# koadman/libMems

Measured on AMD Instinct MI355X. Metric: seed-mers/sec sorted+matched (+ MUMs/sec) at 1/2/4/8 MI355X; HBM GB/s vs roofline, higher is better.
Workload: dtype u64; 1 GPU; BASELINE config 3: 8 x 100 Mbp, seed weight 19 (0x7b974ef), MemHash seed stage (sorted+matched); genomes=8, genome_length=100000000, seedmers_total=799999792, seedmers_rank0=799999792, probes_rank0=100459493, parallelism=1 GPU

## Files before the change

libmems_amd/csrc/mums_internal.h:

```cpp
#pragma once

#include <hip/hip_runtime.h>
#include <stdint.h>
#include <stdlib.h>

#include <vector>

#include "restart_plan.h"

namespace mums {

constexpr int kMaxG = 64;
constexpr int kRepeatLimit = 1000;
constexpr int kBlock = 256;
#ifndef MUMS_SEED_TILE
#define MUMS_SEED_TILE 4096
#endif
constexpr int kSeedTile = MUMS_SEED_TILE;
#ifndef MUMS_SEG_TILE
#define MUMS_SEG_TILE 4096
#endif
constexpr int kSegTile = MUMS_SEG_TILE;
#ifndef MUMS_GROUP_SPLIT
#define MUMS_GROUP_SPLIT 2
#endif
#ifndef MUMS_PROBE_TAKE
#define MUMS_PROBE_TAKE 1984
#endif
constexpr int kProbeSplit = MUMS_GROUP_SPLIT;
constexpr int kProbeTake = MUMS_PROBE_TAKE;
constexpr int kProbeTile = kProbeSplit * kProbeTake;
static_assert(kSegTile % kProbeSplit == 0 && kProbeTake >= 2 && kProbeTake <= kSegTile / kProbeSplit,
              "a probe workgroup takes at most what it stages");
constexpr int kLocalIPT = 16;
constexpr int kMaxMsdBits = 11;
constexpr int kMaxSegBucketBits = 12;

constexpr int kMaxSeedRuns = 16;

struct SeedSpec {
    uint64_t pattern;
    int L;
    int w;
    int nruns;
    int run_start[32];
    int run_len[32];
    int run_dst[32];
    int run_sh[kMaxSeedRuns];
    uint64_t run_mask[kMaxSeedRuns];
};

struct GenomeTable {
    int G;
    uint64_t n[kMaxG];
    uint64_t m[kMaxG];
    uint64_t base[kMaxG + 1];
    uint64_t woff[kMaxG + 1];
    uint32_t tfirst[kMaxG + 1];
    uint32_t gl_shift;
    uint32_t gl_n;
    uint8_t gl[256];
};

inline void genome_lookup_init(GenomeTable& gt) {
    gt.gl_n = 0;
    gt.gl_shift = 0;
    const uint64_t N = gt.base[gt.G];
    if (gt.G < 2 || N == 0 || N >= (1ull << 32)) return;
    if (getenv("MUMS_DEV_NO_GL")) return;
    uint64_t mn = ~0ull;
    for (int g = 0; g < gt.G; ++g) mn = gt.m[g] < mn ? gt.m[g] : mn;
    if (mn == 0) return;
    const int sh = 63 - __builtin_clzll(mn);
    const uint64_t nb = ((N - 1) >> sh) + 1;
    if (nb > 256) return;
    int g = 0;
    for (uint64_t s = 0; s < nb; ++s) {
        const uint64_t i = s << sh;
        while (g + 1 < gt.G && gt.base[g + 1] <= i) ++g;
        gt.gl[s] = (uint8_t)g;
    }
    gt.gl_shift = (uint32_t)sh;
    gt.gl_n = (uint32_t)nb;
}

struct MatchParams {
    uint32_t repeat_tol;
    uint32_t enum_tol;
    uint32_t table_size;
    int masked;
    uint64_t seq_mask;
};

struct DevCounters {
    unsigned long long groups;
    unsigned long long repeat_limit;
    unsigned long long collisions;
    unsigned long long entries;
    uint32_t err;
    uint32_t ntiles;
    uint32_t nprobes;
    uint32_t nmatches;
    uint32_t ngroups;
    uint32_t nchains;
    uint32_t max_bucket;
    uint32_t scratch32;
    unsigned long long walk_words;
    unsigned long long walk_items;
    unsigned long long walk_wins;
    unsigned long long short_words;
    unsigned long long short_items;
    unsigned long long short_wins;
    unsigned long long log_n;
    unsigned long long row_total;
};

struct SegTile {
    uint64_t start;
    uint64_t bstart;
    uint64_t bend;
    uint32_t count;
    uint32_t hbase;
    uint32_t ntb;
    uint32_t tb;
    uint32_t bucket;
    uint32_t order;
};

template <int kBits>
__device__ __forceinline__ uint32_t wave_match_rank_from(uint32_t dg, uint32_t pl, uint32_t ph, uint32_t* peers_out) {
    #pragma unroll
    for (int b = 0; b < kBits; ++b) {
        const uint32_t ms = (uint32_t)__builtin_amdgcn_sbfe((int32_t)dg, b, 1);
        const uint64_t x = __builtin_amdgcn_uicmp(ms, 0u, 33);
        pl = __builtin_amdgcn_bitop3_b32(pl, (uint32_t)x, ms, 0x90);
        ph = __builtin_amdgcn_bitop3_b32(ph, (uint32_t)(x >> 32), ms, 0x90);
    }
    *peers_out = (uint32_t)__builtin_popcount(pl) + (uint32_t)__builtin_popcount(ph);
    return __builtin_amdgcn_mbcnt_hi(ph, __builtin_amdgcn_mbcnt_lo(pl, 0u));
}

template <int kBits>
__device__ __forceinline__ uint32_t wave_match_rank(uint32_t dg, bool valid, uint32_t* peers_out) {
    const uint64_t v = __ballot(valid);
    return wave_match_rank_from<kBits>(dg, (uint32_t)v, (uint32_t)(v >> 32), peers_out);
}

template <int kBits>
__device__ __forceinline__ uint32_t wave_match_rank(uint32_t dg, uint32_t* peers_out) {
    return wave_match_rank_from<kBits>(dg, 0xFFFFFFFFu, 0xFFFFFFFFu, peers_out);
}

__device__ __forceinline__ uint64_t compat_gid(uint64_t k, int kbits) {
    return ((k >> 1) & 0x3FFFFFFFull) | (((k >> kbits) & 1ull) << 30);
}

__device__ __forceinline__ int genome_of(const GenomeTable& gt, uint64_t i) {
    int g = 0;
    #pragma unroll 1
    for (int k = 1; k < gt.G; ++k) g += (i >= gt.base[k]) ? 1 : 0;
    return g;
}

__host__ __device__ inline uint64_t packed_words(uint64_t n) { return (2 * n) / 32 + (((2 * n) % 32) ? 1 : 0) + 2; }

hipError_t launch_seed_pack(const SeedSpec& ss, const GenomeTable& gt, const char* const* d_ascii,
                            uint32_t* d_packed, int mode, bool key64, void* d_ckey, int msd_bits,
                            uint32_t* d_hist, uint32_t ntiles, uint32_t* d_err, hipStream_t st);
hipError_t launch_seed_scatter(const SeedSpec& ss, const GenomeTable& gt, const uint32_t* d_packed, int msd_bits,
                               const uint32_t* d_hist_scanned, uint32_t ntiles, uint64_t* d_rec, hipStream_t st,
                               uint8_t* d_side = nullptr, int side_bits = 0);
hipError_t launch_seed_scatter_chunk(const SeedSpec& ss, const GenomeTable& gt, const uint32_t* d_packed, int msd_bits,
                                     const uint32_t* d_hist_slice, uint32_t ntiles, uint32_t dlo, uint32_t nbc,
                                     uint64_t* d_rec, hipStream_t st, const uint64_t* d_cbase = nullptr, int mb = 0,
                                     uint8_t* d_side = nullptr, int side_bits = 0);
size_t msd_split_tmp_bytes(uint64_t n, int parent_bits);
hipError_t msd_split(const uint64_t* rin, const uint8_t* side, uint64_t* rout, uint64_t n, int parent_bits, int S,
                     const uint32_t* bstart_in, uint32_t* bstart_out, void* d_tmp, hipStream_t st);
hipError_t launch_keys_of_genome(const SeedSpec& ss, const uint32_t* d_words, uint64_t m, uint64_t* d_out,
                                 hipStream_t st, bool ref_form = true);

size_t scan_tmp_bytes(uint64_t n);
hipError_t exclusive_scan_u32(uint32_t* d_data, uint64_t n, void* d_tmp, uint32_t* d_total, hipStream_t st);
hipError_t launch_sum_u64(const uint32_t* d_data, uint64_t n, unsigned long long* d_total, hipStream_t st);

size_t radix_tmp_bytes(uint64_t n);
template <typename K>
hipError_t radix_sort(const K* keys_in, const uint32_t* vals_in, uint64_t n, int bits,
                      K* kA, uint32_t* vA, K* kB, uint32_t* vB, void* d_tmp, int* out_buf,
                      hipStream_t st, hipEvent_t* ev_ds = nullptr);

uint64_t seg_tiles_upper(uint64_t n, int msd_bits, uint32_t tile = kSegTile);
size_t seg_tmp_bytes(uint64_t n, int msd_bits);
hipError_t launch_regroup(const uint64_t* src, uint64_t* dst, const uint64_t* d_chunks, uint32_t nchunks, uint64_t n,
                          hipStream_t st);
hipError_t seg_bucket_starts(const uint32_t* d_hist_scanned, uint32_t T, int msd_bits, uint64_t n, uint32_t* bstart,
                             hipStream_t st);
hipError_t build_seg_tiles_from_starts(const uint32_t* bstart, int msd_bits, uint64_t n, SegTile* d_tiles,
                                       uint32_t* d_ntiles, void* d_tmp, hipStream_t st, uint32_t tile = kSegTile);
hipError_t build_seg_tiles(const uint32_t* d_hist_scanned, uint32_t T, int msd_bits, uint64_t n, SegTile* d_tiles,
                           uint32_t* d_ntiles, uint32_t* d_bstart, void* d_tmp, hipStream_t st);
hipError_t seg_radix_sort(uint64_t* recA, uint64_t* recB, uint64_t n, int key_bits, const SegTile* d_tiles,
                          uint64_t ntiles_ub, void* d_tmp, int* out_buf, hipStream_t st,
                          hipEvent_t* ev_ds = nullptr);
size_t onesweep_tmp_bytes(uint64_t n, int msd_bits, int key_bits);
hipError_t seg_onesweep_sort(uint64_t* recA, uint64_t* recB, uint64_t n, int key_bits, int msd_bits,
                             const uint32_t* d_bstart, void* d_tmp, uint32_t* d_err, int* out_buf, hipStream_t st,
                             hipEvent_t* ev_ds = nullptr, int key_shift = 32, bool mask_parity = false,
                             bool key_runs = false, const uint32_t* hist_in = nullptr,
                             const uint64_t* gsrc = nullptr, uint32_t* gout = nullptr);
size_t seg_parity_fix_tmp_bytes(uint64_t n);
hipError_t seg_parity_fix(uint64_t* rec, uint64_t* scratch, uint64_t n, int key_bits, int msd_bits,
                          const uint32_t* d_bstart, void* d_tmp, uint32_t* d_err, hipStream_t st, int key_shift = 32);
int seg_onesweep_launches(int key_bits);
bool seg_wide_sort_enabled();
int seg_wide_passes(int key_bits);
size_t onesweep_wide_tmp_bytes(uint64_t n, int msd_bits, int key_bits);
hipError_t seg_onesweep_sort_wide(uint64_t* recA, uint64_t* recB, uint64_t n, int key_bits, int msd_bits,
                                  const uint32_t* d_bstart, void* d_tmp, uint32_t* d_err, int* out_buf,
                                  hipStream_t st, hipEvent_t* ev_ds, int key_shift = 32);

inline uint64_t group_tiles_upper(uint64_t n, int msd_bits) { return seg_tiles_upper(n, msd_bits, kProbeTile); }
uint64_t group_slot_count(uint64_t ntiles);
uint64_t group_blocks(uint64_t ntiles, bool packed);
template <int MG, typename View>
hipError_t launch_probe_tiles(View v, const SegTile* tiles, uint64_t ntiles, uint64_t N, const GenomeTable& gt,
                              const MatchParams& mp, int L, uint32_t* tile_count, uint64_t* slot_info,
                              uint32_t* slot_bucket, void* counters, hipStream_t st);
hipError_t launch_probe_compact(uint64_t nblocks, const uint32_t* tile_count, const uint32_t* tile_off,
                                const uint64_t* slot_info, const uint32_t* slot_bucket, uint64_t* probe_info,
                                uint32_t* probe_bucket, hipStream_t st, bool packed);
template <int MG, typename View>
hipError_t launch_materialize(View v, const uint64_t* probe_info, uint64_t P, const GenomeTable& gt,
                              const MatchParams& mp, int L, int64_t* rows, hipStream_t st, uint64_t* lkey = nullptr,
                              uint32_t* fsk = nullptr, uint32_t* lhash = nullptr, int32_t* rows32 = nullptr);
hipError_t launch_row_buckets(const int64_t* rows, uint64_t P, int G, uint32_t table_size, const uint32_t* d_bounds,
                              uint32_t nranks, uint32_t* out, hipStream_t st);
hipError_t launch_gather_rows(const int64_t* src, const uint32_t* perm, uint64_t P, int G, int64_t* dst,
                              hipStream_t st);
hipError_t launch_rec_pairs(const uint64_t* rec, uint64_t n, const uint32_t* d_bst, uint32_t nb, uint32_t kfirst,
                            int kb_rec, uint64_t* key, uint32_t* idx, hipStream_t st);
hipError_t launch_rec_pairs33(const uint64_t* rec, uint64_t n, const uint32_t* d_bst, uint32_t nb, uint32_t kfirst,
                              int kb_rec, uint64_t* key, uint64_t* idx, hipStream_t st);
hipError_t launch_chain_dest(const uint32_t* fk, uint64_t nch, const uint32_t* pdest, uint32_t* cdest, hipStream_t st);
hipError_t launch_inverse_perm(const uint32_t* perm, uint64_t n, uint32_t* inv, hipStream_t st);
hipError_t launch_chain_tags(const uint32_t* chain_of, const uint32_t* perm, const uint32_t* sdest, uint64_t P,
                             const uint32_t* cinv, const uint32_t* cstart, uint32_t* tags, hipStream_t st);
hipError_t launch_chain_entries_out(const int64_t* pool, const uint32_t* fk, const uint32_t* cperm,
                                    const uint32_t* scdest, uint64_t nch, int G, const uint32_t* pinv,
                                    const uint32_t* rstart, int64_t* eout, uint32_t* fout, hipStream_t st);
hipError_t launch_kept_dest(const int64_t* rows, uint64_t P, int G, const uint32_t* chain_of, const uint32_t* cinv,
                            const uint2* thr, const uint32_t* fk, const uint32_t* pdest, uint32_t nranks, uint32_t* dest,
                            hipStream_t st);
hipError_t launch_dest_first(const uint32_t* sdest, uint64_t P, uint32_t* first, hipStream_t st);
hipError_t launch_entry_first(const uint32_t* scdest, uint64_t nch, const uint32_t* rcount, const uint32_t* perm,
                              const uint32_t* sdest, uint64_t K, const uint32_t* chain_of, const uint32_t* cinv,
                              const uint32_t* rstart, uint32_t* efirst, hipStream_t st);
hipError_t launch_flat_tiles(uint64_t N, SegTile* d_tiles, hipStream_t st, bool packed = false);
inline uint64_t flat_group_tiles(uint64_t N, bool packed) {
    const uint64_t tile = packed ? kProbeTile : kSegTile;
    return (N + tile - 1) / tile;
}

hipError_t launch_bucket_ranges(const uint32_t* sb, uint64_t P, uint32_t* bstart, uint32_t* bend, uint32_t* d_max,
                                hipStream_t st);
template <int MG, typename View>
hipError_t launch_replay_kept(View v, const GenomeTable& gt, const MatchParams& mp, int L, uint64_t P,
                              const int64_t* pool, const uint32_t* chain_of, const uint32_t* fk, uint32_t nch,
                              void* d_tmp, void* d_radix_tmp, void* d_scan_tmp, uint32_t lds_cap, uint32_t* tsize,
                              void* ctr, uint64_t* dbg, hipStream_t st, uint64_t* mlog, uint32_t** tbl_out,
                              const uint32_t** base_out, void* (*alloc)(void*, size_t), void* alloc_ctx,
                              const uint32_t* jl = nullptr);
template <int MG, typename View>
hipError_t launch_replay_carried(View v, const GenomeTable& gt, const MatchParams& mp, int L, uint64_t P,
                                 const int64_t* pool, uint32_t C, const uint32_t* kcnt, uint32_t nch,
                                 const uint32_t* jl, uint32_t lds_max, uint32_t* tsize, void* ctr, hipStream_t st,
                                 uint64_t* mlog, uint32_t** tbl_out, const uint32_t** base_out,
                                 void* (*alloc)(void*, size_t), void* alloc_ctx);
hipError_t launch_keep_pack(const uint64_t* len, const int64_t* s, uint64_t M, int G, int64_t* pool, hipStream_t st);
}
struct mums_ctx;
namespace mums {
hipStream_t ctx_stream(mums_ctx* ctx);
int ctx_device(mums_ctx* ctx);
int ctx_table_genomes(mums_ctx* ctx, uint32_t* table_size, uint32_t* genomes);
uint32_t ctx_repeat_tol(mums_ctx* ctx);
bool ctx_merge_chunked(mums_ctx* ctx);
bool ctx_tie_all(mums_ctx* ctx);
bool ctx_pcompat(mums_ctx* ctx);
int ctx_compat_layout(mums_ctx* ctx, uint32_t* first, uint32_t* nown, std::vector<uint64_t>* lens);
int ctx_compat_rank_find(mums_ctx* ctx, const char* const* d_ascii, const uint64_t* lens, int G, uint32_t rank,
                         uint32_t ranks, int stage);
int ctx_compat_rank_export(mums_ctx* ctx, uint64_t* bucket_counts, int64_t* d_rows, uint64_t* M);
int ctx_compat_rank_merge(mums_ctx* ctx, const int64_t* d_rows, uint32_t W, const uint64_t* counts, uint32_t nb);

struct EoWork {
    void *K = nullptr, *V = nullptr, *V2 = nullptr, *fl = nullptr, *fr = nullptr, *Lpos = nullptr, *Rpos = nullptr;
    void *bound = nullptr, *segA = nullptr, *segB = nullptr, *act = nullptr, *heap = nullptr, *piv = nullptr;
    void *nsw = nullptr, *scratch = nullptr, *plen = nullptr, *ps = nullptr, *nm_key = nullptr, *nm_id = nullptr;
    void *nk2 = nullptr, *nv2 = nullptr, *nk3 = nullptr, *nv3 = nullptr, *radix = nullptr, *ctr = nullptr;
    uint64_t cap_n = 0, cap_pool = 0, cap_new = 0, pool_n = 0, n_final = 0;
    int pool_G = 0;
    unsigned long long hbuf[8] = {};
    EoWork() = default;
    EoWork(const EoWork&) = delete;
    EoWork& operator=(const EoWork&) = delete;
    ~EoWork();
    void release();
};
hipError_t eliminate_overlaps_device(EoWork& w, const uint64_t* d_len, const int64_t* d_s, uint64_t M, int G,
                                     uint64_t* M_out, hipStream_t st);
hipError_t eliminate_overlaps_v2_device(EoWork& w, const uint64_t* d_len, const int64_t* d_s, uint64_t M, int G,
                                        const uint32_t* seq_ids, uint32_t nids, bool eliminate_both, uint64_t* M_out,
                                        hipStream_t st);
hipError_t eo_gather(EoWork& w, int G, uint64_t* d_len_out, int64_t* d_s_out, hipStream_t st);
hipError_t eo_sort_ids(EoWork& w, const uint64_t* d_keys, uint32_t n, int depth_override, uint32_t* d_ids_out,
                       hipStream_t st);

size_t chain_tmp_bytes(uint64_t P, uint32_t Tb, int G);
hipError_t launch_add_offset(uint32_t* a, uint64_t n, uint32_t off, hipStream_t st);
size_t chain_merge_tmp_bytes(uint64_t n);
size_t chain_thr_tmp_bytes(uint64_t n);
hipError_t launch_chain_thresholds(const int64_t* entries, uint64_t n, const GenomeTable& gt, const MatchParams& mp,
                                   int64_t* pool_out, void* d_tmp, void* d_radix_tmp, void* d_scan_tmp,
                                   uint32_t* d_nchains, uint32_t* h_nchains, uint2* thr, hipStream_t st);
hipError_t launch_chain_merge(const int64_t* pool_loc, uint64_t n, int G, uint32_t* chain_of, uint64_t P,
                              int64_t* pool_out, void* d_tmp, void* d_radix_tmp, void* d_scan_tmp, uint32_t* d_nchains,
                              hipStream_t st, const uint32_t* fk_loc, uint32_t* fk_out);
size_t chain_radix_tmp_bytes(uint64_t P);
template <int MG, typename View>
hipError_t launch_chains(View v, const uint64_t* probe_info, uint64_t P, const GenomeTable& gt, const MatchParams& mp,
                         const SeedSpec& ss, const uint32_t* packed, void* d_chain_tmp, void* d_scan_tmp,
                         void* d_radix_tmp, uint32_t* chain_of, int64_t* pool, uint32_t* d_nchains, hipStream_t st,
                         void* ctr, hipEvent_t* ev_walk, uint32_t* fk, uint32_t kbase, bool lkey_ready = false,
                         uint32_t* jl = nullptr);
uint64_t* chain_lkey_slot(void* d_chain_tmp, uint64_t P, int G);
bool chain_line_records(uint64_t P, const GenomeTable& gt);
void chain_line_slots(void* d_chain_tmp, uint64_t P, int G, uint64_t** rec, uint32_t** lhash);
hipError_t launch_emit(const uint32_t* obase, const uint32_t* bstart, const uint32_t* tbl, const int64_t* pool, int G,
                       uint32_t table_size, uint64_t M, uint64_t* out_len, int64_t* out_s, hipStream_t st);

size_t occ_tmp_bytes(uint64_t m);
hipError_t launch_seed_occurrence(const uint64_t* sk, const uint32_t* sv, uint64_t m, uint64_t n, int L, void* d_tmp,
                                  float* out, hipStream_t st);
hipError_t launch_unpack(const uint32_t* words, uint64_t n, char* out, hipStream_t st);
size_t filter_tmp_bytes(uint64_t M);
hipError_t launch_match_filter(const uint64_t* len, const int64_t* s, uint64_t M, int G, uint32_t mult,
                               uint64_t min_len, void* d_tmp, uint32_t* d_kept, uint64_t* len2, int64_t* s2,
                               hipStream_t st);

template <typename View>
hipError_t launch_pairwise_count(View v, uint64_t N, const GenomeTable& gt, uint32_t* npairs, void* ctr,
                                 hipStream_t st);
template <typename View>
hipError_t launch_pairwise_emit(View v, uint64_t N, const GenomeTable& gt, int L, const uint32_t* npairs,
                                const uint32_t* off, int64_t* rows, hipStream_t st);

hipError_t launch_digit_totals(const uint32_t* hist, uint32_t ndigits, uint32_t T, unsigned long long* out,
                               hipStream_t st);

template <typename View>
hipError_t launch_enum_count(View v, uint64_t N, const GenomeTable& gt, const MatchParams& mp, uint32_t* ncalls,
                             void* ctr, hipStream_t st);
template <typename View>
hipError_t launch_enum_emit(View v, uint64_t N, const GenomeTable& gt, const MatchParams& mp, int L,
                            const uint32_t* ncalls, const uint32_t* off, uint64_t P, int64_t* rows, hipStream_t st);

hipError_t launch_chunk_pairs(const uint64_t* rec, uint64_t n, const uint32_t* bstart, uint32_t nb, uint64_t digit0,
                              uint64_t* key, uint64_t* idx, hipStream_t st);

hipError_t launch_genome_keys(uint64_t* ckey, uint64_t N, const GenomeTable& gt, int kbits, hipStream_t st);
hipError_t launch_compat_breaks(const uint64_t* sk, const GenomeTable& gt, uint64_t kmask, int mx, uint64_t chunk,
                                uint64_t* cs, uint64_t* bm, uint32_t cap, uint32_t* d_nch, uint32_t* err,
                                hipStream_t st);
hipError_t launch_compat_find(const uint64_t* sk, const GenomeTable& gt, uint64_t kmask, int mx, int L, uint64_t* cs,
                              const uint64_t* bm, uint32_t nch, hipStream_t st);
hipError_t launch_compat_chunk_keys(const uint64_t* sk, const uint32_t* sv, uint64_t N, const GenomeTable& gt,
                                    int kbits, const uint64_t* cs, uint32_t nch, uint64_t* key2, uint32_t* val2,
                                    uint64_t* ck, hipStream_t st);
hipError_t launch_compat_cands(const uint64_t* key2, uint64_t N, uint64_t* list, unsigned long long* cnt, uint64_t cap,
                               hipStream_t st);
hipError_t launch_compat_fire(const restart::PlanData& d, const uint64_t* key2, uint64_t N, int kbits,
                              const uint64_t* cand, uint64_t C, const uint64_t* cs, uint32_t nch, uint32_t* out,
                              uint64_t* cend, uint64_t* cons, hipStream_t st);
hipError_t launch_compat_strip(const uint64_t* in, uint64_t* out, uint64_t n, uint64_t mask, hipStream_t st);
hipError_t launch_compat_recs(const uint64_t* key2, const uint32_t* idx, uint64_t n, int kbits, uint64_t* rec,
                              uint32_t* clash, uint32_t* scratch, void* scan_tmp, bool force_scan, uint64_t* list,
                              unsigned long long* cnt, uint64_t cap, hipStream_t st);
hipError_t launch_compat_split(const uint64_t* sk, const GenomeTable& gt, const uint64_t* cs, uint32_t nch,
                               uint32_t* out, hipStream_t st);
hipError_t launch_compat_probe_chunks(const uint64_t* probe_info, uint64_t P, const uint64_t* key2, int kbits,
                                      uint32_t nch, uint32_t* pfirst, hipStream_t st);
hipError_t launch_compat_drop(const uint64_t* k_in, const uint32_t* v_in, uint64_t N, const uint64_t* rlo,
                              const uint64_t* rhi, const uint64_t* rpre, uint32_t R, uint64_t* k_out, uint32_t* v_out,
                              hipStream_t st);
hipError_t launch_compat_merge(uint32_t* tsize, const uint32_t* bstart, uint32_t* tbl, const int64_t* pool, int G,
                               uint32_t Tb, unsigned long long* collisions, const uint32_t* tscan, uint64_t total,
                               uint32_t* first_fail, hipStream_t st);
hipError_t launch_compat_merge_from(uint32_t* tsize, const uint32_t* bstart, uint32_t* tbl, const int64_t* pool, int G,
                                    uint32_t nb, const uint32_t* first_fail, unsigned long long* collisions,
                                    hipStream_t st);
hipError_t launch_compat_chunk_span(const uint64_t* key2, uint64_t n, int kbits, uint32_t c0, uint32_t c1,
                                    uint64_t* out, hipStream_t st);

hipError_t launch_rank_rows(const uint32_t* obase, const uint32_t* bstart, const uint32_t* tbl, const int64_t* pool,
                            int G, uint32_t Tb, uint64_t M, int64_t* rows, hipStream_t st);
hipError_t launch_rank_lb(const int64_t* pool, int G, uint32_t nA, const uint32_t* offA, const uint32_t* offB,
                          uint32_t nb, uint32_t nB, uint32_t* lbA, uint32_t* nd, uint32_t* bad, hipStream_t st);
hipError_t launch_rank_place(const int64_t* pool, int G, uint32_t nA, const uint32_t* offA, const uint32_t* offB,
                             uint32_t nb, uint32_t nB, const uint32_t* lbA, const uint32_t* ndp, uint32_t* catoff,
                             uint32_t* tsize, uint32_t* tblcat, hipStream_t st);
hipError_t launch_rank_check(const int64_t* pool, int G, const uint32_t* catoff, const uint32_t* tsize, uint32_t nb,
                             uint32_t ncat, const uint32_t* tblcat, uint32_t* bad, hipStream_t st);
hipError_t launch_rank_exact_init(uint32_t nA, const uint32_t* offA, const uint32_t* offB, const uint32_t* catoff,
                                  uint32_t nb, uint32_t ncat, const uint32_t* bad, uint32_t* tblcat, uint32_t* tsize,
                                  uint32_t* first_fail, hipStream_t st);
hipError_t launch_rank_gather(const int64_t* pool, int G, const uint32_t* catoff, const uint32_t* tsize, uint32_t nb,
                              uint32_t ncat, const uint32_t* tblcat, const uint32_t* newoff, int64_t* out,
                              hipStream_t st);
hipError_t launch_rank_list(const int64_t* rows, int G, uint64_t M, uint64_t* out_len, int64_t* out_s, hipStream_t st);

struct RsStream {
    int kind;
    const uint64_t* rec;
    const uint32_t* bstart;
    int B, kbits;
    const void* key;
    const uint32_t* idx;
};
struct RestartWs {
    uint64_t* ckf;
    uint64_t* ck;
    uint32_t* gen;
    uint32_t* inv;
    uint32_t *kA, *kB, *vA, *vB;
    uint64_t* dm;
    uint64_t* dbase;
    void* tmp;
    size_t bytes;
};
RestartWs restart_ws_layout(void* base, uint64_t n, int G);
size_t restart_ws_bytes(uint64_t n, int G);
hipError_t launch_restart_smls(const RsStream& s, uint64_t n, const GenomeTable& gt, const RestartWs& w,
                               hipStream_t st);
hipError_t launch_restart_cands(const RestartWs& w, uint64_t n, uint64_t* d_list, unsigned long long* d_cnt,
                                uint64_t cap, hipStream_t st);
hipError_t launch_restart_plan(const RestartWs& w, int G, const uint64_t* d_cand, uint64_t C, uint64_t* d_pre,
                               uint64_t* d_S, restart::PlanOut* d_out, hipStream_t st);
hipError_t launch_restart_dpre(const restart::PlanData& d, const uint64_t* d_cand, uint64_t C, uint64_t* d_pre,
                               unsigned* cbad, hipStream_t st);
hipError_t launch_restart_dplan(const restart::PlanData& d, const uint64_t* d_cand, uint64_t C, const uint64_t* d_pre,
                                const unsigned* cbad, uint64_t* d_S, restart::PlanOut* d_out, hipStream_t st);
hipError_t launch_tie_heads(const RestartWs& w, int G, const uint64_t* gk, const uint64_t* gu, const uint32_t* gp,
                            const uint64_t* Sall, uint64_t ng, int* ord, hipStream_t st);
hipError_t launch_restart_compact(const RsStream& s, uint64_t n, int G, const RestartWs& w, const uint64_t* d_rkey,
                                  uint64_t R, const uint64_t* d_rS, const uint64_t* d_S0, void* dst_a, uint32_t* dst_idx,
                                  uint32_t* dst_bstart, uint32_t* d_total, hipStream_t st);

hipError_t launch_map_starts(const uint32_t* bstart, uint32_t nb, const uint32_t* pos, uint32_t* out, hipStream_t st);

struct CrStream {
    const uint64_t* rec;
    const uint64_t* dstart;
    uint32_t nd;
    uint64_t N;
    uint32_t kb = 31, ib = 33;
};
uint64_t cr_blocks(uint64_t N);
hipError_t launch_cr_counts(const CrStream& s, const GenomeTable& gt, uint32_t* gcnt, void* d_scan_tmp, hipStream_t st);
hipError_t launch_cr_partition(const CrStream& s, const GenomeTable& gt, const uint32_t* gscan, int kbits, uint64_t* sk,
                               uint32_t* sv, uint64_t* ck, hipStream_t st);
size_t cr_chunk_part_cnt_words(uint64_t N, uint32_t nch);
bool cr_chunk_part_fits(uint64_t N, uint32_t nch);
hipError_t launch_cr_chunk_part(const CrStream& s, const GenomeTable& gt, const uint32_t* gscan, const uint64_t* cs,
                                uint32_t nch, int kbits, uint32_t* cnt, void* d_scan_tmp, uint64_t* key2, uint32_t* idx,
                                hipStream_t st);
hipError_t launch_compat_fast_chunks(const CrStream& s, const GenomeTable& gt, const uint32_t* gscan, int mx,
                                    uint64_t chunk, int L, uint32_t nch, uint64_t* cs, uint32_t* flags, hipStream_t st);
size_t cr_direct_ws_bytes(uint64_t N);
hipError_t launch_cr_compat_direct(const CrStream& s, const GenomeTable& gt, const uint32_t* gscan, const uint64_t* cs,
                                   uint32_t nch, int kbits, uint64_t* rec, uint64_t* k2, uint8_t* sc, void* ws,
                                   uint32_t* flags, hipStream_t st);
hipError_t launch_cr_ck(const CrStream& s, const GenomeTable& gt, const uint32_t* gscan, uint64_t* ck, hipStream_t st,
                        const uint64_t* lbase = nullptr);
hipError_t launch_cr_query(const CrStream& s, const GenomeTable& gt, const uint32_t* gscan, const uint64_t* q, uint64_t nq,
                           uint64_t* out, hipStream_t st);
hipError_t launch_cr_ck_query(const uint64_t* ck, const GenomeTable& gt, const uint64_t* q, uint64_t nq, uint64_t* out,
                              hipStream_t st);
hipError_t launch_cr_cands(const CrStream& s, uint64_t* list, unsigned long long* cnt, uint64_t cap, hipStream_t st);
hipError_t launch_cr_runs(const uint64_t* ck, const GenomeTable& gt, const uint64_t* sp, uint64_t rows, uint64_t* runs,
                          unsigned long long* nr, uint64_t cap, hipStream_t st);
hipError_t launch_cr_kpos(const CrStream& s, const GenomeTable& gt, int g, uint64_t* K, hipStream_t st);
hipError_t launch_cr_pair_flags(const uint64_t* ck, int G, const uint64_t* lbase, const uint64_t* gofs, uint64_t n,
                                uint32_t* out, hipStream_t st);
hipError_t launch_cr_tie_vals(const CrStream& s, const GenomeTable& gt, const uint32_t* gscan, const uint64_t* vofs,
                              const uint32_t* V, uint64_t* rec, hipStream_t st);
hipError_t launch_cr_tie_all(const CrStream& s, const GenomeTable& gt, const uint32_t* gscan, int g, const uint32_t* ts,
                             const uint32_t* V, uint64_t* rec, hipStream_t st);
hipError_t launch_cr_druns(const uint64_t* ck, int G, const uint64_t* lbase, const uint64_t* goff, const uint64_t* gn,
                           const uint64_t* sp, uint64_t rows, uint64_t* runs, unsigned long long* nr, uint64_t cap,
                           hipStream_t st);
hipError_t launch_cr_dtie_write(const CrStream& s, const GenomeTable& gt, const uint64_t* runs, uint64_t nrun,
                                const uint64_t* ck, const uint64_t* lbase, const uint64_t* goff, const uint32_t* V,
                                const uint64_t* vofs, uint64_t* rec, hipStream_t st);
hipError_t launch_cr_tie_write(const CrStream& s, const GenomeTable& gt, int g, const uint64_t* runs, uint64_t nrun,
                               const uint64_t* ck, const uint32_t* V, uint64_t* rec, hipStream_t st);
hipError_t launch_cr_live_compact(const CrStream& s, const GenomeTable& gt, const uint32_t* gscan, uint64_t lo,
                                  uint64_t hi, const uint64_t* rkey, uint64_t R, const uint64_t* rS, const uint64_t* S0,
                                  uint32_t* live, uint32_t* pos, void* d_scan_tmp, uint64_t* dst,
                                  const uint32_t* bstart, uint32_t nb, uint32_t* dst_bstart, uint32_t* d_total,
                                  hipStream_t st, const uint64_t* goff = nullptr);

hipError_t launch_batch_gap(const char* ascii, uint64_t lo, uint64_t hi, unsigned long long* d_first, hipStream_t st);
hipError_t launch_batch_keys(const char* ascii, const uint64_t* aoff, const uint32_t* mbase, uint32_t nseg, uint32_t G,
                             uint32_t N, const SeedSpec& ss, int kbits, uint64_t* keys, hipStream_t st);
struct BatchReplay {
    const uint64_t* sk;
    const uint32_t* sv;
    const uint64_t* keys;
    const uint32_t* mbase;
    const uint64_t* nlen;
    const uint32_t* order;
    uint64_t* ord;
    int64_t* pool;
    uint32_t pool_cap;
    uint32_t* pool_n;
    uint32_t *cnt, *probes, *coll, *flag;
    uint32_t B, G;
    int L, kbits;
    uint32_t table_size;
    int masked;
    uint64_t seq_mask;
    const uint32_t* ord_base = nullptr;
    const uint32_t* ord_cap = nullptr;
};
hipError_t launch_batch_replay(const BatchReplay& b, hipStream_t st);
hipError_t launch_batch_emit(const uint64_t* ord, const int64_t* pool, const uint32_t* mbase, const uint32_t* cnt,
                             const uint64_t* doff, uint32_t B, uint32_t G, uint64_t* out_len, int64_t* out_s,
                             hipStream_t st);

hipError_t launch_anchor_gather(const uint64_t* ord, const uint32_t* obase, const int64_t* pool, const uint64_t* toff,
                                uint32_t B, uint32_t G, int64_t* wlen, int64_t* ws, hipStream_t st,
                                const uint32_t* nrow = nullptr);
struct AnchorTail {
    uint64_t* K;
    uint32_t* V;
    int64_t* wlen;
    int64_t* ws;
    const uint64_t* toff;
    const uint32_t* order;
    const uint8_t* skip;
    uint32_t* cnt;
    uint32_t B, G;
    int eliminate_both;
    uint64_t min_length;
};
hipError_t launch_anchor_tail(const AnchorTail& a, hipStream_t st);
hipError_t launch_anchor_emit(const uint32_t* V, const int64_t* wlen, const int64_t* ws, const uint64_t* toff,
                              const uint32_t* cnt, const uint64_t* doff, uint32_t B, uint32_t G, uint64_t* out_len,
                              int64_t* out_s, hipStream_t st);

uint64_t recursion_slice_rows(uint64_t n, uint32_t G);
struct RecursionTail {
    uint64_t* K;
    uint32_t* V;
    int64_t* wlen;
    int64_t* ws;
    const uint64_t* soff;
    const uint32_t* nrow;
    const uint32_t* order;
    const uint8_t* skip;
    uint32_t* cnt;
    uint32_t* flag;
    uint32_t B, G;
    uint32_t multiplicity;
    uint64_t min_length;
};
hipError_t launch_recursion_tail(const RecursionTail& a, hipStream_t st);

struct TieWs {
    uint64_t n;
    int G;
    uint64_t smax;
    uint32_t* pf;
    uint32_t* ts;
    uint64_t* K;
    uint32_t* V;
    uint32_t *fl, *fr, *Lpos, *Rpos;
    uint8_t* bound;
    void *segA, *segB, *heap;
    uint32_t *act, *off, *nsw, *ctr;
    uint64_t* piv;
    uint64_t *dbase, *dm;
    void* tmp;
    size_t bytes;
};
TieWs tie_ws_layout(void* base, uint64_t n, int G);
size_t tie_ws_bytes(uint64_t n, int G);
hipError_t tie_set_genomes(const TieWs& w, const uint64_t* base, const uint64_t* m, hipStream_t st);
hipError_t tie_clear_flags(const TieWs& w, hipStream_t st);
hipError_t tie_mark_all(const TieWs& w, const uint64_t* ck, hipStream_t st);
hipError_t tie_mark_starts(const TieWs& w, const uint64_t* ck, const uint64_t* d_sp, uint64_t rows, hipStream_t st);
hipError_t tie_scatter_keys(const TieWs& w, const uint64_t* ckf, const uint64_t* rec, const uint32_t* idx,
                            hipStream_t st);
hipError_t tie_prepare(const TieWs& w, uint64_t* flagged, hipStream_t st);
hipError_t tie_replay(const TieWs& w, hipStream_t st);
hipError_t tie_writeback(const TieWs& w, uint64_t* rec, uint32_t* idx, const uint32_t* inv, hipStream_t st);
hipError_t tie_slots_out(const TieWs& w, uint32_t* out, hipStream_t st);

}
```

libmems_amd/csrc/radix_sort.hip:

```cpp
#include <cstdlib>
#include "mums_internal.h"

namespace mums {

namespace {

constexpr int kRTile = 4096;
constexpr int kRounds = kRTile / kBlock;
constexpr int kWaves = kBlock / 64;
constexpr int kDigits = 256;

template <typename K>
__global__ __launch_bounds__(kBlock) void rs_upsweep(const K* __restrict__ keys, uint64_t n, int shift,
                                                     uint32_t* __restrict__ hist, uint32_t nblocks) {
    __shared__ uint32_t h[kWaves][kDigits];
    const int lane = threadIdx.x & 63, wv = threadIdx.x >> 6;
    for (int i = threadIdx.x; i < kWaves * kDigits; i += kBlock) (&h[0][0])[i] = 0;
    __syncthreads();
    const uint64_t b0 = (uint64_t)blockIdx.x * kRTile + (uint64_t)wv * (kRTile / kWaves);
    #pragma unroll 4
    for (int r = 0; r < kRounds; ++r) {
        const uint64_t i = b0 + (uint64_t)r * 64 + lane;
        const bool valid = i < n;
        const uint32_t d = valid ? (uint32_t)(keys[i] >> shift) & 0xFFu : 0u;
        uint32_t tot;
        const uint32_t rk = wave_match_rank<8>(d, valid, &tot);
        if (valid && rk == 0) atomicAdd(&h[wv][d], tot);
    }
    __syncthreads();
    const int t = threadIdx.x;
    uint32_t s = 0;
    #pragma unroll
    for (int w = 0; w < kWaves; ++w) s += h[w][t];
    hist[(uint64_t)t * nblocks + blockIdx.x] = s;
}

template <typename K, bool kImplicitVals>
__global__ __launch_bounds__(kBlock) void rs_downsweep(const K* __restrict__ kin, const uint32_t* __restrict__ vin,
                                                       uint64_t n, int shift, const uint32_t* __restrict__ hist,
                                                       uint32_t nblocks, K* __restrict__ kout,
                                                       uint32_t* __restrict__ vout) {
    __shared__ K skeys[kRTile];
    __shared__ uint32_t svals[kRTile];
    __shared__ uint32_t wcnt[kWaves][kDigits];
    __shared__ uint32_t lstart[kDigits];
    __shared__ uint32_t gofs[kDigits];
    __shared__ uint32_t s_w[kWaves];
    const int lane = threadIdx.x & 63, wv = threadIdx.x >> 6;
    for (int i = threadIdx.x; i < kWaves * kDigits; i += kBlock) (&wcnt[0][0])[i] = 0;
    __syncthreads();

    const uint64_t tile0 = (uint64_t)blockIdx.x * kRTile;
    const uint64_t b0 = tile0 + (uint64_t)wv * (kRTile / kWaves);
    K key[kRounds];
    uint32_t val[kRounds];
    uint32_t rank[kRounds];
    #pragma unroll
    for (int r = 0; r < kRounds; ++r) {
        const uint64_t i = b0 + (uint64_t)r * 64 + lane;
        const bool valid = i < n;
        key[r] = valid ? kin[i] : (K)0;
        val[r] = kImplicitVals ? (uint32_t)i : (valid ? vin[i] : 0u);
        const uint32_t d = (uint32_t)(key[r] >> shift) & 0xFFu;
        uint32_t tot;
        const uint32_t rk = wave_match_rank<8>(d, valid, &tot);
        uint32_t old = 0;
        if (valid) old = wcnt[wv][d];
        if (valid && rk == 0) wcnt[wv][d] = old + tot;
        rank[r] = old + rk;
    }
    __syncthreads();

    {
        const int t = threadIdx.x;
        uint32_t acc = 0;
        #pragma unroll
        for (int w = 0; w < kWaves; ++w) {
            uint32_t c = wcnt[w][t];
            wcnt[w][t] = acc;
            acc += c;
        }
        uint32_t v = acc;
        #pragma unroll
        for (int d = 1; d < 64; d <<= 1) {
            uint32_t x = __shfl_up(v, d, 64);
            if (lane >= d) v += x;
        }
        if (lane == 63) s_w[wv] = v;
        __syncthreads();
        uint32_t wpre = 0;
        #pragma unroll
        for (int w = 0; w < kWaves; ++w) wpre += (w < wv) ? s_w[w] : 0u;
        lstart[t] = wpre + v - acc;
        gofs[t] = hist[(uint64_t)t * nblocks + blockIdx.x];
    }
    __syncthreads();

    #pragma unroll
    for (int r = 0; r < kRounds; ++r) {
        const uint64_t i = b0 + (uint64_t)r * 64 + lane;
        if (i < n) {
            const uint32_t d = (uint32_t)(key[r] >> shift) & 0xFFu;
            const uint32_t lp = lstart[d] + wcnt[wv][d] + rank[r];
            skeys[lp] = key[r];
            svals[lp] = val[r];
        }
    }
    __syncthreads();

    const uint64_t cnt = (n - tile0) < (uint64_t)kRTile ? (n - tile0) : (uint64_t)kRTile;
    #pragma unroll
    for (int r = 0; r < kRounds; ++r) {
        const uint32_t s = threadIdx.x + r * kBlock;
        if (s < cnt) {
            const K k = skeys[s];
            const uint32_t d = (uint32_t)(k >> shift) & 0xFFu;
            const uint64_t o = (uint64_t)gofs[d] + (s - lstart[d]);
            kout[o] = k;
            vout[o] = svals[s];
        }
    }
}

uint64_t tiles(uint64_t n) { return (n + kRTile - 1) / kRTile; }

}

size_t radix_tmp_bytes(uint64_t n) {
    uint64_t h = (uint64_t)kDigits * tiles(n);
    return (h + 64) * sizeof(uint32_t) + scan_tmp_bytes(h) + 256;
}

template <typename K>
hipError_t radix_sort(const K* keys_in, const uint32_t* vals_in, uint64_t n, int bits, K* kA, uint32_t* vA,
                      K* kB, uint32_t* vB, void* d_tmp, int* out_buf, hipStream_t st, hipEvent_t* ev_ds) {
    const int passes = (bits + 7) / 8;
    *out_buf = (passes - 1) % 2;
    if (n == 0 || passes == 0) return hipSuccess;
    const uint32_t nb = (uint32_t)tiles(n);
    uint32_t* hist = (uint32_t*)d_tmp;
    void* stmp = (void*)(hist + (uint64_t)kDigits * nb + 64);
    const K* ksrc = keys_in;
    const uint32_t* vsrc = vals_in;
    for (int p = 0; p < passes; ++p) {
        K* kdst = (p % 2 == 0) ? kA : kB;
        uint32_t* vdst = (p % 2 == 0) ? vA : vB;
        const int shift = 8 * p;
        hipLaunchKernelGGL(rs_upsweep<K>, dim3(nb), dim3(kBlock), 0, st, ksrc, n, shift, hist, nb);
        hipError_t e = exclusive_scan_u32(hist, (uint64_t)kDigits * nb, stmp, nullptr, st);
        if (e != hipSuccess) return e;
        if (ev_ds) (void)hipEventRecord(ev_ds[2 * p], st);
        if (vsrc == nullptr)
            hipLaunchKernelGGL((rs_downsweep<K, true>), dim3(nb), dim3(kBlock), 0, st, ksrc, vsrc, n, shift, hist,
                               nb, kdst, vdst);
        else
            hipLaunchKernelGGL((rs_downsweep<K, false>), dim3(nb), dim3(kBlock), 0, st, ksrc, vsrc, n, shift, hist,
                               nb, kdst, vdst);
        e = hipGetLastError();
        if (e != hipSuccess) return e;
        if (ev_ds) (void)hipEventRecord(ev_ds[2 * p + 1], st);
        ksrc = kdst;
        vsrc = vdst;
    }
    return hipSuccess;
}

template hipError_t radix_sort<uint32_t>(const uint32_t*, const uint32_t*, uint64_t, int, uint32_t*, uint32_t*,
                                         uint32_t*, uint32_t*, void*, int*, hipStream_t, hipEvent_t*);
template hipError_t radix_sort<uint64_t>(const uint64_t*, const uint32_t*, uint64_t, int, uint64_t*, uint32_t*,
                                         uint64_t*, uint32_t*, void*, int*, hipStream_t, hipEvent_t*);

}
```

Before: 41.39 billion seed-mers/s.

## Use run-length counting in radix upsweep and streamline downsweep offsets

The upsweep histogram now uses a DPP neighbour compare and a ballot to count runs of equal digits, replacing the per-digit wave match rank. It also batches key loads eight at a time, with separate paths for full and partial tiles. The downsweep loads all keys up front and pads invalid entries in the partial tile with all-ones keys so the ranking loop needs no validity checks. It folds the local start and global offset into a single per-digit delta held in shared memory. This lowers ALU and LDS work per key, but on random digits most runs have length one, so the upsweep may issue more LDS atomics.

```diff
diff --git a/libmems_amd/csrc/mums_internal.h b/libmems_amd/csrc/mums_internal.h
--- a/libmems_amd/csrc/mums_internal.h
+++ b/libmems_amd/csrc/mums_internal.h
@@ -149,6 +149,21 @@
 template <int kBits>
 __device__ __forceinline__ uint32_t wave_match_rank(uint32_t dg, uint32_t* peers_out) {
     return wave_match_rank_from<kBits>(dg, 0xFFFFFFFFu, 0xFFFFFFFFu, peers_out);
+}
+
+__device__ __forceinline__ void wave_count_runs(uint32_t* __restrict__ hw, uint32_t dg, int lane, int nvalid) {
+    const uint32_t pd = (uint32_t)__builtin_amdgcn_update_dpp((int)dg, (int)dg, 0x138, 0xF, 0xF, false);
+    const bool valid = lane < nvalid;
+    const bool head = valid && (lane == 0 || pd != dg);
+    const uint64_t hm = __ballot(head);
+    const uint64_t vm = nvalid >= 64 ? ~0ull : ((1ull << nvalid) - 1);
+    if (hm == vm) {
+        if (valid) atomicAdd(&hw[dg], 1u);
+    } else if (head) {
+        const uint64_t above = (hm >> 1) >> lane;
+        const int len = above ? __builtin_ctzll(above) + 1 : nvalid - lane;
+        atomicAdd(&hw[dg], (uint32_t)len);
+    }
 }
 
 __device__ __forceinline__ uint64_t compat_gid(uint64_t k, int kbits) {
diff --git a/libmems_amd/csrc/radix_sort.hip b/libmems_amd/csrc/radix_sort.hip
--- a/libmems_amd/csrc/radix_sort.hip
+++ b/libmems_amd/csrc/radix_sort.hip
@@ -9,6 +9,8 @@
 constexpr int kRounds = kRTile / kBlock;
 constexpr int kWaves = kBlock / 64;
 constexpr int kDigits = 256;
+
+constexpr int kUpBatch = 8;
 
 template <typename K>
 __global__ __launch_bounds__(kBlock) void rs_upsweep(const K* __restrict__ keys, uint64_t n, int shift,
@@ -17,15 +19,32 @@
     const int lane = threadIdx.x & 63, wv = threadIdx.x >> 6;
     for (int i = threadIdx.x; i < kWaves * kDigits; i += kBlock) (&h[0][0])[i] = 0;
     __syncthreads();
-    const uint64_t b0 = (uint64_t)blockIdx.x * kRTile + (uint64_t)wv * (kRTile / kWaves);
-    #pragma unroll 4
-    for (int r = 0; r < kRounds; ++r) {
-        const uint64_t i = b0 + (uint64_t)r * 64 + lane;
-        const bool valid = i < n;
-        const uint32_t d = valid ? (uint32_t)(keys[i] >> shift) & 0xFFu : 0u;
-        uint32_t tot;
-        const uint32_t rk = wave_match_rank<8>(d, valid, &tot);
-        if (valid && rk == 0) atomicAdd(&h[wv][d], tot);
+    const uint64_t tile0 = (uint64_t)blockIdx.x * kRTile;
+    const K* __restrict__ kw = keys + tile0 + (uint32_t)wv * (kRTile / kWaves) + lane;
+    if (n - tile0 >= (uint64_t)kRTile) {
+        #pragma unroll
+        for (int r0 = 0; r0 < kRounds; r0 += kUpBatch) {
+            K kk[kUpBatch];
+            #pragma unroll
+            for (int u = 0; u < kUpBatch; ++u) kk[u] = kw[(r0 + u) * 64];
+            #pragma unroll
+            for (int u = 0; u < kUpBatch; ++u)
+                wave_count_runs(h[wv], (uint32_t)(kk[u] >> shift) & 0xFFu, lane, 64);
+        }
+    } else {
+        const int cnt = (int)(n - tile0) - wv * (kRTile / kWaves);
+        #pragma unroll 1
+        for (int r0 = 0; r0 < kRounds && r0 * 64 < cnt; r0 += kUpBatch) {
+            K kk[kUpBatch];
+            #pragma unroll
+            for (int u = 0; u < kUpBatch; ++u) kk[u] = (r0 + u) * 64 + lane < cnt ? kw[(r0 + u) * 64] : (K)0;
+            #pragma unroll
+            for (int u = 0; u < kUpBatch; ++u) {
+                const int nv = cnt - (r0 + u) * 64;
+                if (nv <= 0) break;
+                wave_count_runs(h[wv], (uint32_t)(kk[u] >> shift) & 0xFFu, lane, nv < 64 ? nv : 64);
+            }
+        }
     }
     __syncthreads();
     const int t = threadIdx.x;
@@ -43,42 +62,55 @@
     __shared__ K skeys[kRTile];
     __shared__ uint32_t svals[kRTile];
     __shared__ uint32_t wcnt[kWaves][kDigits];
-    __shared__ uint32_t lstart[kDigits];
-    __shared__ uint32_t gofs[kDigits];
+    __shared__ uint32_t gdelta[kDigits];
     __shared__ uint32_t s_w[kWaves];
     const int lane = threadIdx.x & 63, wv = threadIdx.x >> 6;
     for (int i = threadIdx.x; i < kWaves * kDigits; i += kBlock) (&wcnt[0][0])[i] = 0;
     __syncthreads();
 
     const uint64_t tile0 = (uint64_t)blockIdx.x * kRTile;
-    const uint64_t b0 = tile0 + (uint64_t)wv * (kRTile / kWaves);
+    const uint32_t cnt = (n - tile0) < (uint64_t)kRTile ? (uint32_t)(n - tile0) : (uint32_t)kRTile;
+    const bool full = cnt == (uint32_t)kRTile;
+    const uint32_t w0 = (uint32_t)wv * (kRTile / kWaves) + lane;
+    const K* __restrict__ kt = kin + tile0;
     K key[kRounds];
     uint32_t val[kRounds];
     uint32_t rank[kRounds];
+    if (full) {
+        #pragma unroll
+        for (int r = 0; r < kRounds; ++r) key[r] = kt[w0 + r * 64];
+        if (!kImplicitVals) {
+            #pragma unroll
+            for (int r = 0; r < kRounds; ++r) val[r] = vin[tile0 + w0 + r * 64];
+        }
+    } else {
+        #pragma unroll
+        for (int r = 0; r < kRounds; ++r) key[r] = w0 + r * 64 < cnt ? kt[w0 + r * 64] : ~(K)0;
+        if (!kImplicitVals) {
+            #pragma unroll
+            for (int r = 0; r < kRounds; ++r) val[r] = w0 + r * 64 < cnt ? vin[tile0 + w0 + r * 64] : 0u;
+        }
+    }
     #pragma unroll
     for (int r = 0; r < kRounds; ++r) {
-        const uint64_t i = b0 + (uint64_t)r * 64 + lane;
-        const bool valid = i < n;
-        key[r] = valid ? kin[i] : (K)0;
-        val[r] = kImplicitVals ? (uint32_t)i : (valid ? vin[i] : 0u);
+        if (kImplicitVals) val[r] = (uint32_t)tile0 + w0 + r * 64;
         const uint32_t d = (uint32_t)(key[r] >> shift) & 0xFFu;
         uint32_t tot;
-        const uint32_t rk = wave_match_rank<8>(d, valid, &tot);
-        uint32_t old = 0;
-        if (valid) old = wcnt[wv][d];
-        if (valid && rk == 0) wcnt[wv][d] = old + tot;
+        const uint32_t rk = wave_match_rank<8>(d, &tot);
+        const uint32_t old = wcnt[wv][d];
+        if (rk == 0) wcnt[wv][d] = old + tot;
         rank[r] = old + rk;
     }
     __syncthreads();
 
     {
         const int t = threadIdx.x;
+        uint32_t c[kWaves];
         uint32_t acc = 0;
         #pragma unroll
         for (int w = 0; w < kWaves; ++w) {
-            uint32_t c = wcnt[w][t];
-            wcnt[w][t] = acc;
-            acc += c;
+            c[w] = acc;
+            acc += wcnt[w][t];
         }
         uint32_t v = acc;
         #pragma unroll
@@ -91,33 +123,41 @@
         uint32_t wpre = 0;
         #pragma unroll
         for (int w = 0; w < kWaves; ++w) wpre += (w < wv) ? s_w[w] : 0u;
-        lstart[t] = wpre + v - acc;
-        gofs[t] = hist[(uint64_t)t * nblocks + blockIdx.x];
+        const uint32_t lstart = wpre + v - acc;
+        #pragma unroll
+        for (int w = 0; w < kWaves; ++w) wcnt[w][t] = lstart + c[w];
+        gdelta[t] = hist[(uint64_t)t * nblocks + blockIdx.x] - lstart;
     }
     __syncthreads();
 
     #pragma unroll
     for (int r = 0; r < kRounds; ++r) {
-        const uint64_t i = b0 + (uint64_t)r * 64 + lane;
-        if (i < n) {
-            const uint32_t d = (uint32_t)(key[r] >> shift) & 0xFFu;
-            const uint32_t lp = lstart[d] + wcnt[wv][d] + rank[r];
-            skeys[lp] = key[r];
-            svals[lp] = val[r];
-        }
-    }
-    __syncthreads();
-
-    const uint64_t cnt = (n - tile0) < (uint64_t)kRTile ? (n - tile0) : (uint64_t)kRTile;
-    #pragma unroll
-    for (int r = 0; r < kRounds; ++r) {
-        const uint32_t s = threadIdx.x + r * kBlock;
-        if (s < cnt) {
+        const uint32_t d = (uint32_t)(key[r] >> shift) & 0xFFu;
+        const uint32_t lp = wcnt[wv][d] + rank[r];
+        skeys[lp] = key[r];
+        svals[lp] = val[r];
+    }
+    __syncthreads();
+
+    if (full) {
+        #pragma unroll
+        for (int r = 0; r < kRounds; ++r) {
+            const uint32_t s = threadIdx.x + r * kBlock;
             const K k = skeys[s];
-            const uint32_t d = (uint32_t)(k >> shift) & 0xFFu;
-            const uint64_t o = (uint64_t)gofs[d] + (s - lstart[d]);
+            const uint32_t o = gdelta[(uint32_t)(k >> shift) & 0xFFu] + s;
             kout[o] = k;
             vout[o] = svals[s];
+        }
+    } else {
+        #pragma unroll
+        for (int r = 0; r < kRounds; ++r) {
+            const uint32_t s = threadIdx.x + r * kBlock;
+            if (s < cnt) {
+                const K k = skeys[s];
+                const uint32_t o = gdelta[(uint32_t)(k >> shift) & 0xFFu] + s;
+                kout[o] = k;
+                vout[o] = svals[s];
+            }
         }
     }
 }
```

After: 41.74 billion seed-mers/s (median of 5 runs). Within noise of the previous version (+0.9%).
